# jerry102102102/RL_brain_trainer

Measured on AMD Instinct MI355X. Metric: env-steps/sec (whole node), Stage-5 Approach->Finisher PPO loops (rollout + update); value = the Approach loop, finisher.value = the Finisher loop, higher is better.
Workload: dtype f32

## Files before the change

### include/kp1_ppo.h

```cpp
#ifndef KP1_PPO_H
#define KP1_PPO_H

#include <stdint.h>

#include "kp1.h"

#ifdef __cplusplus
extern "C" {
#endif

int kp1_gae_scan(int32_t device, const float* rewards, const float* values, const uint8_t* dones, const float* last_values,
                 float gamma, float gae_lambda, float* advantages, float* returns, int32_t T, int32_t N, void* stream);

int kp1_gae_scan_replicas(int32_t device, const float* rewards, const float* values, const uint8_t* dones, const float* last_values,
                          const float* gamma_lambda, int32_t n_per_replica, float* advantages, float* returns, int32_t T, int32_t N, void* stream);

int kp1_bootstrap_truncated(int32_t device, float* rewards, const float* terminal_values, const uint8_t* dones, float gamma,
                            int64_t count, void* stream);

int kp1_adv_minibatch_sums(int32_t device, const float* advantages, const int64_t* idx, int64_t total, int64_t minibatch, double* out_sums,
                           void* stream);
int kp1_random_permutation(int32_t device, int64_t n, const uint32_t* keys, int64_t* out, void* stream);

int kp1_adv_minibatch_stats(int32_t device, const double* sums, int64_t n_minibatches, float* out_stats, void* stream);
// ... 56 lines not shown
typedef struct kp1_dock_curriculum_state {
  int32_t stage_index, stage_episode_count, ring_len, ring_head, window_episodes, n_stages, n_events, reserved0;
  int64_t num_timesteps;
  kp1_dock_curriculum_stage stages[KP1_DOCK_CURRICULUM_MAX_STAGES];
  kp1_dock_curriculum_event events[KP1_DOCK_CURRICULUM_MAX_HISTORY];
  uint8_t ring[KP1_DOCK_CURRICULUM_MAX_WINDOW];
} kp1_dock_curriculum_state;
int kp1_dock_curriculum_create(kp1_env* env, const kp1_dock_curriculum_stage* stages_host, int32_t n_stages, int32_t window_episodes,
                               kp1_dock_curriculum_state** out_dev);
int kp1_dock_curriculum_destroy(kp1_env* env, kp1_dock_curriculum_state* st_dev);
int kp1_dock_curriculum_observe(kp1_env* env, kp1_dock_curriculum_state* st_dev, const uint8_t* dones, int32_t n_local, int32_t chunk_steps, int32_t world,
                                void* stream);
int kp1_dock_curriculum_read(kp1_env* env, const kp1_dock_curriculum_state* st_dev, kp1_dock_curriculum_state* out_host, void* stream);
int kp1_dock_curriculum_create_population(kp1_env* env, const kp1_dock_curriculum_stage* stages_host, int32_t n_stages, int32_t window_episodes,
                                          int32_t n_replicas, kp1_dock_curriculum_state** out_dev);
int kp1_dock_curriculum_observe_population(kp1_env* env, kp1_dock_curriculum_state* states_dev, const uint8_t* dones, int32_t n_per_replica,
                                           int32_t n_replicas, void* stream);
int kp1_dock_curriculum_read_replica(kp1_env* env, const kp1_dock_curriculum_state* states_dev, int32_t n_replicas, int32_t k,
                                     kp1_dock_curriculum_state* out_host, void* stream);

#define KP1_MLP_IN 56
#define KP1_MLP_IN_PAD 64
#define KP1_MLP_IN_ROUTE 80
#define KP1_MLP_IN_ROUTE_PAD 128
#define KP1_MLP_ACT 7

typedef struct kp1_mlp kp1_mlp;

int kp1_mlp_create(int32_t device, int32_t hidden, int32_t max_batch, kp1_mlp** out);
int kp1_mlp_create_ex(int32_t device, int32_t hidden, int32_t obs_dim, int32_t max_batch, kp1_mlp** out);
#define KP1_MLP_MAX_REPLICAS 16
int kp1_mlp_create_population(int32_t device, int32_t hidden, int32_t obs_dim, int32_t max_batch, int32_t replicas, kp1_mlp** out);
int32_t kp1_mlp_replicas(const kp1_mlp* m);
typedef struct kp1_replica_hparams {
  float learning_rate, adam_eps, max_grad_norm, clip_range, ent_coef, vf_coef;
} kp1_replica_hparams;
int kp1_mlp_set_replica_hparams(kp1_mlp* m, const kp1_replica_hparams* host, int32_t n, void* stream);
int kp1_mlp_destroy(kp1_mlp* m);
int64_t kp1_mlp_num_params(int32_t hidden);
int64_t kp1_mlp_num_params_ex(int32_t hidden, int32_t obs_dim);
int kp1_mlp_pack_weights(kp1_mlp* m, const float* params, void* stream);

int kp1_mlp_forward(kp1_mlp* m, const float* obs, int32_t obs_stride, int32_t n, const float* noise, float* mean, float* value,
                    float* action, float* clipped_action, float* log_prob, void* stream);

int kp1_mlp_forward_env_step(kp1_mlp* m, kp1_env* env, const float* obs, int32_t obs_stride, const float* noise, float* value, float* action,
                             float* log_prob, float* next_obs, float* reward, uint8_t* done, float* terminal_obs, void* stream);

int kp1_eval_step(kp1_mlp* m, kp1_env* env, float* obs, float* reward, uint8_t* done, const kp1_eval_buffers* buffers, int32_t step,
                  const double* ready_thresholds , int32_t confirm_steps, void* stream);

#define KP1_EVAL_EPISODES_MAX_STEPS 256
int kp1_eval_episodes(kp1_mlp* m, kp1_env* env, float* obs, float* reward, uint8_t* done, const kp1_eval_buffers* buffers,
                      int32_t first_step, int32_t last_step, const double* ready_thresholds , int32_t confirm_steps, void* stream);

int kp1_mlp_loss_grad(kp1_mlp* m, const float* obs, int32_t obs_stride, const int64_t* idx, int32_t n, const float* actions,
                      const float* old_log_prob, const float* advantages, const float* returns, float adv_mean, float adv_inv_std,
                      const float* adv_stats_dev, float clip_range, float ent_coef, float vf_coef, float inv_count, float* grad_out,
                      float* stats_out, int32_t grad_is_zero, void* stream);

#define KP1_MLP_OPT_FUSED 1
#define KP1_MLP_OPT_ACTOR_EXTRA_STEPS 2
#define KP1_MLP_OPT_STEP_COUNT 3
#define KP1_MLP_OPT_PROFILE 4
#define KP1_MLP_OPT_BF16X3_WGRAD 5
#define KP1_MLP_PROFILE_SLOTS 4
#define KP1_MLP_PROFILE_TILE 0
#define KP1_MLP_PROFILE_WGRAD 1
#define KP1_MLP_PROFILE_FINALIZE 2
#define KP1_MLP_PROFILE_ADAM 3
int kp1_mlp_set_option(kp1_mlp* m, int32_t option, int32_t value);
int kp1_mlp_profile_read(kp1_mlp* m, float* out_us , int32_t* out_launches );

int kp1_mlp_adam_step(kp1_mlp* m, float* params, float* grad, float* exp_avg, float* exp_avg_sq, float lr, float eps,
                      float max_grad_norm, int32_t step, int32_t flags, void* stream);

int kp1_mlp_anchor_loss_grad(kp1_mlp* m, const float* obs, int32_t obs_stride, const int64_t* idx, int32_t n, const float* teacher_actions,
                             float loss_weight, float* grad_out, float* loss_out, void* stream);

int kp1_mlp_anchor_adam_step(kp1_mlp* m, float* params, float* grad, float* exp_avg, float* exp_avg_sq, float lr, float eps,
                             float max_grad_norm, int32_t step, void* stream);

int kp1_mlp_placement_check(int32_t device, int32_t n_rows, int32_t* out, void* stream);
int kp1_mlp_time_kernels(kp1_mlp* m, const float* obs, int32_t obs_stride, int32_t n, int32_t iters, float* out_ms, double* out_flops,
                         void* stream);

int kp1_set_obs_stride(kp1_env* env, int32_t stride);

#ifdef __cplusplus
}
#endif
#endif
```

### rl_brain_trainer_amd/csrc/kp1_mlp.hip

```cpp
#include <hip/hip_runtime.h>
#include <hip/hip_ext.h>

#include <cmath>
#include <cstddef>
#include <cstdlib>
#include <cstring>
#include <limits>
#include <vector>

#include "../../include/kp1_ppo.h"
#include "../../include/kp1_route.h"
#include "../../include/kp1_ziggurat_tables.h"
#include "kp1_device.hpp"
#include "kp1_host.hpp"

using kp1::fail;
using namespace kp1;

typedef float f32x16 __attribute__((ext_vector_type(16)));
typedef float f32x4 __attribute__((ext_vector_type(4)));

namespace {

constexpr int ACT = KP1_MLP_ACT, HEADS = 8;
// ... 1173 lines not shown

struct AnchorFinalizeArgs {
  FinalizeArgs f;
  float* loss_out;
};

template <bool POP = false>
__global__ void __launch_bounds__(256) anchor_finalize_kernel(const AnchorFinalizeArgs a_) {
  const FinalizeArgs a = POP ? finalize_args_replica(a_.f, blockIdx.y) : a_.f;
  const ParamLayout& L = a.L;
  __shared__ double sq[4];
  const int64_t i = (int64_t)(blockIdx.x * 256u + threadIdx.x);
  float gval = 0.f;
  if (i < L.total) {
    if (is_actor_element(L, i)) {
      const PartialSrc s = finalize_source(a, i);
      for (int c = 0; c < s.n; ++c) gval += s.p[(int64_t)c * s.stride];
    }
    a.grad[i] = gval;
  }
  if (blockIdx.x == 0 && threadIdx.x == 0) {
    float t = 0.f;
    for (int c = 0; c < a.h_n; ++c) t += a.hpart[(int64_t)c * a.h_stride + 10 * L.Hp + 15];
    a_.loss_out[POP ? blockIdx.y : 0u] = t;
  }
  double w = (double)gval * (double)gval;
  for (int off = 32; off > 0; off >>= 1) w += __shfl_xor(w, off);
  if ((threadIdx.x & 63) == 0) sq[threadIdx.x >> 6] = w;
  __syncthreads();
  if (threadIdx.x == 0) a.sumsq[blockIdx.x] = ((sq[0] + sq[1]) + sq[2]) + sq[3];
}

template <bool POP = false>
__global__ void __launch_bounds__(ADAM_BLOCK) anchor_adam_kernel(float* __restrict__ p, const float* __restrict__ g, float* __restrict__ m, float* __restrict__ v,
                                                          const double* __restrict__ partials, int n_partials, float lr, float eps, float max_norm,
                                                          const ParamLayout L, const Packed k_, const int* __restrict__ step_dev, int host_step,
                                                          unsigned r_partials, const float* __restrict__ hparams) {
  __shared__ float sh[3];
  const Packed k = POP ? packed_replica(k_, L, blockIdx.y) : k_;
  if constexpr (POP) {
    const unsigned o = blockIdx.y * (unsigned)L.total;
    p += o; g += o; m += o; v += o;
    partials += blockIdx.y * r_partials;
    if (hparams) {
      const float* e = hparams + blockIdx.y * (unsigned)HP_FIELDS;
      lr = e[HP_LR];
      eps = e[HP_EPS];
    }
  }
  const int64_t i = (int64_t)blockIdx.x * ADAM_BLOCK + threadIdx.x;
  const bool actor = i < L.total && is_actor_element(L, i);
  const int64_t il = actor ? i : L.p_w1;
  const float g_in = g[il], m_in = m[il], v_in = v[il], p_in = p[il];
  double s = 0.0;
  if (threadIdx.x < 64) {
    for (int q = threadIdx.x; q < n_partials; q += 64) s += partials[q];
    for (int off = 32; off > 0; off >>= 1) s += __shfl_xor(s, off);
  }
  if (threadIdx.x == 0) {
    const float norm = (float)sqrt(s);
    const int st = (host_step > 0 ? host_step : step_dev[0]) + step_dev[1] + 1;
    sh[0] = max_norm > 0.f ? fminf(max_norm / (norm + 1e-6f), 1.f) : 1.f;
    sh[1] = (float)((double)lr / (1.0 - pow(0.9, (double)st)));
    sh[2] = (float)sqrt(1.0 - pow(0.999, (double)st));
  }
  __syncthreads();
  if (actor) {
    const float gi = g_in * sh[0];
    const float mn = 0.9f * m_in + 0.1f * gi;
    const float vn = 0.999f * v_in + 0.001f * gi * gi;
    const float denom = sqrtf(vn) / sh[2] + eps;
    const float pn = p_in - sh[1] * (mn / denom);
    m[i] = mn; v[i] = vn; p[i] = pn;
    pack_one(i, pn, L, k);
  }
}

__global__ void anchor_count_kernel(int* __restrict__ actor_extra) { *actor_extra += 1; }

#include "kp1_env_step.inc"
#include "kp1_eval_step.inc"
#include "kp1_rollout_step.inc"
#include "kp1_mlp_tile.inc"
#include "kp1_mlp_fused.inc"
#include "kp1_route_step.inc"
#include "kp1_route_rollout_step.inc"
#include "kp1_route_chain_step.inc"

}

#include "kp1_route_host.hpp"

struct kp1_mlp {
  int device = 0, H = 0, Hp = 0, max_batch = 0;
  int K = 1;
  ParamLayout L;
  Packed k{};
  float* h1 = nullptr;
  float* h2 = nullptr;
  float* dz2 = nullptr;
  float* dz1 = nullptr;
  float* xf = nullptr;
  int bf16x3 = 0;
  unsigned short* sp_h1 = nullptr; unsigned short* sp_dz2 = nullptr; unsigned short* sp_dz1 = nullptr; unsigned short* sp_xf = nullptr;
  double* partials = nullptr;
  double* anchor_partials = nullptr;
  float* slab = nullptr;
  float* slab1 = nullptr;
  float* bslab = nullptr;
  float* hpart = nullptr;
  int n_finalize_blocks = 0;
  int* step_dev = nullptr;
  float* hparams_dev = nullptr;
  bool hparams_on = false;
  int last_s2_n = 0, last_s1_n = 0;
  int fused = 1;
  const float* last_params = nullptr;
  bool slab_stale = false;
  std::vector<void*> allocs;
  int profile = 0;
  struct ProfPair { hipEvent_t a, b; };
  std::vector<ProfPair> prof[KP1_MLP_PROFILE_SLOTS];
  int prof_used[KP1_MLP_PROFILE_SLOTS] = {0, 0, 0, 0};
};

namespace {
struct ProfSlotInFlight { hipEvent_t a = nullptr, b = nullptr; bool attached = false; };
thread_local ProfSlotInFlight tl_prof;

struct ProfScope {
  kp1_mlp* m; int slot; hipStream_t stream; bool on;
  ProfScope(kp1_mlp* m_, int slot_, hipStream_t s_) : m(m_), slot(slot_), stream(s_), on(m_->profile != 0) {
    if (!on) return;
    auto& v = m->prof[slot];
    if (m->prof_used[slot] >= (int)v.size()) {
      kp1_mlp::ProfPair p{};
      if (hipEventCreate(&p.a) != hipSuccess || hipEventCreate(&p.b) != hipSuccess) { on = false; return; }
      v.push_back(p);
    }
    tl_prof.a = v[m->prof_used[slot]].a;
    tl_prof.b = v[m->prof_used[slot]].b;
    tl_prof.attached = false;
  }
  ~ProfScope() {
    if (!on) return;
    if (!tl_prof.attached) {
      (void)hipEventRecord(tl_prof.a, stream);
      (void)hipEventRecord(tl_prof.b, stream);
    }
    tl_prof = ProfSlotInFlight{};
    m->prof_used[slot] += 1;
  }
};

#define KP1_LAUNCH(kernel, grid, block, bytes, stream, ...)                                                        \
  do {                                                                                                             \
    if (tl_prof.a != nullptr && !tl_prof.attached) {                                                               \
      tl_prof.attached = true;                                                                                     \
      hipExtLaunchKernelGGL(kernel, grid, block, bytes, stream, tl_prof.a, tl_prof.b, 0, __VA_ARGS__);             \
    } else {                                                                                                       \
      hipLaunchKernelGGL(kernel, grid, block, bytes, stream, __VA_ARGS__);                                         \
    }                                                                                                              \
  } while (0)
}

namespace {
// ... 1007 lines not shown
        if (launch_nt<EPI_DTANH>(g, stream) != KP1_OK) return KP1_ERR_NO_DEVICE;
      } else if (which == 2) {
        GemmTN t{};
        t.B = n; t.chunk = tn_chunk_rows(n, (Hp / 128) * (Hp / 128) * 2);
        t.D = m->dz2; t.ldd = Hp; t.strideD = act_stride; t.X = m->h1; t.ldx = Hp; t.strideX = act_stride;
        t.Nload = Hp; t.n_i_tiles = Hp / 128;
        if (launch_tn(m, t, Hp / 128, Hp, m->slab, nullptr, stream) != KP1_OK) return KP1_ERR_NO_DEVICE;
      } else if (which == 3) {
        g.A = obs; g.lda = obs_stride; g.strideA = 0; g.W = m->k.w1p; g.strideW = (int64_t)Hp * INP; g.bias = m->k.b1; g.strideBias = Hp;
        g.C = m->h1; g.K = INP; g.Kreal = obs_stride >= INP ? INP : IN;
        if (launch_nt<EPI_BIAS_TANH>(g, stream) != KP1_OK) return KP1_ERR_NO_DEVICE;
      } else if (which == 4) {
        FusedArgs fa{};
        fa.obs = obs; fa.obs_stride = obs_stride; fa.Kreal = obs_stride >= INP ? INP : IN; fa.inp = INP; fa.idx = nullptr; fa.n = n;
        fa.k = m->k;
        fa.actions = m->h2; fa.old_logp = m->h2 + (int64_t)ACT * n; fa.adv = m->h2 + (int64_t)(ACT + 1) * n; fa.ret = m->h2 + (int64_t)(ACT + 2) * n;
        fa.adv_mode = 3; fa.adv_mean = 0.f; fa.adv_inv_std = 1.f;
        fa.clip_range = 0.2f; fa.vf_coef = 0.5f; fa.inv_count = 1.f / n;
        fa.h1 = m->h1; fa.dz2 = m->dz2; fa.dz1 = m->dz1; fa.act_stride = act_stride; fa.xf = m->xf;
        fa.bslab = m->bslab; fa.hpart = m->hpart; fa.hpart_stride = 10 * Hp + 32;
        if (launch_fused(fa, stream) != KP1_OK) return KP1_ERR_NO_DEVICE;
      } else {
        TnFragArgs t{};
    t.inp = INP;
        t.dz2 = m->dz2; t.h1 = m->h1; t.dz1 = m->dz1; t.act_stride = act_stride; t.xf = m->xf;
        t.slab2 = m->slab; t.s2_net = (int64_t)Hp * Hp; t.s2_chunk = 2 * t.s2_net;
        t.slab1 = m->slab1; t.s1_net = (int64_t)Hp * INP; t.s1_chunk = 2 * t.s1_net;
        t.groups = (n + FU_BM - 1) / FU_BM * (FU_BM / 8);
        t.cg2 = ((t.groups + TN_SPLIT2 - 1) / TN_SPLIT2 + 7) / 8 * 8;
        t.cg1 = ((t.groups + TN_SPLIT1 - 1) / TN_SPLIT1 + 7) / 8 * 8;
        t.n_chunks2 = (t.groups + t.cg2 - 1) / t.cg2;
        t.n_chunks1 = (t.groups + t.cg1 - 1) / t.cg1;
        if (launch_tn_frag(t, stream) != KP1_OK) return KP1_ERR_NO_DEVICE;
      }
    }
    HIP_TRY(hipEventRecord(e1, stream));
    HIP_TRY(hipEventSynchronize(e1));
    float ms = 0.f;
    HIP_TRY(hipEventElapsedTime(&ms, e0, e1));
    out_ms[which] = ms / iters;
    return KP1_OK;
  };
  for (int which : {3, 0, 1, 2}) {
    rc = time_it(which);
    if (rc != KP1_OK) return rc;
  }
  out_ms[4] = out_ms[5] = 0.f;
  out_flops[4] = out_flops[5] = 0.0;
  if (Hp == FU_HP) {
    for (int which : {4, 5}) {
      rc = time_it(which);
      if (rc != KP1_OK) return rc;
    }
  }
  const double M = n, H = Hp;
  out_flops[0] = 2.0 * 2.0 * M * H * H;
  out_flops[1] = 2.0 * 2.0 * M * H * H;
  out_flops[2] = 2.0 * 2.0 * M * H * H;
  out_flops[3] = 2.0 * 2.0 * M * H * INP;
  if (Hp == FU_HP) {
    out_flops[4] = 2.0 * 2.0 * M * (H * (double)INP + 2.0 * H * H);
    out_flops[5] = 2.0 * 2.0 * M * (H * H + H * (double)INP);
  }
  (void)hipEventDestroy(e0);
  (void)hipEventDestroy(e1);
  return KP1_OK;
}

__global__ void __launch_bounds__(FU_NTH, 2) placement_probe_kernel(unsigned int* __restrict__ where, unsigned int* __restrict__ arrived, unsigned int total) {
  extern __shared__ float lds[];
  if (threadIdx.x == 0) {
    const unsigned int hw = __builtin_amdgcn_s_getreg((31 << 11) | 4);
    const unsigned int xcc = __builtin_amdgcn_s_getreg((3 << 11) | 20);
    const unsigned int linear = blockIdx.x + gridDim.x * blockIdx.z;
    where[linear] = (xcc << 16) | (((hw >> 13) & 7u) << 8) | (((hw >> 12) & 1u) << 4) | ((hw >> 8) & 15u);
    lds[0] = 0.f;
    __hip_atomic_fetch_add(arrived, 1u, __ATOMIC_RELAXED, __HIP_MEMORY_SCOPE_AGENT);
    const unsigned long long t0 = wall_clock64();
    while (__hip_atomic_load(arrived, __ATOMIC_RELAXED, __HIP_MEMORY_SCOPE_AGENT) < total && wall_clock64() - t0 < 200000ull) __builtin_amdgcn_s_sleep(8);
  }
  __syncthreads();
}

int kp1_mlp_placement_check(int32_t device, int32_t n_rows, int32_t* out, void* stream_) {
  if (!out || n_rows <= 0) return fail(KP1_ERR_INVALID, "bad argument to kp1_mlp_placement_check");
  HIP_TRY(hipSetDevice(device));
  hipStream_t stream = (hipStream_t)stream_;
  int n_cus = 0;
  HIP_TRY(hipDeviceGetAttribute(&n_cus, hipDeviceAttributeMultiprocessorCount, device));
  const dim3 grid((n_rows + FU_BM - 1) / FU_BM, 1, 2);
  const unsigned int total = grid.x * grid.z;
  if ((int)total > 2 * n_cus) return fail(KP1_ERR_UNSUPPORTED, "placement probe: the grid must be resident at once");
  unsigned int* dev = nullptr;
  HIP_TRY(hipMalloc(&dev, sizeof(unsigned int) * (total + 1)));
  HIP_TRY(hipMemsetAsync(dev, 0, sizeof(unsigned int) * (total + 1), stream));
  const size_t bytes = sizeof(float) * FU_LDS_FLOATS;
  HIP_TRY(hipFuncSetAttribute((const void*)placement_probe_kernel, hipFuncAttributeMaxDynamicSharedMemorySize, (int)bytes));
  hipLaunchKernelGGL(placement_probe_kernel, grid, dim3(FU_NTH), bytes, stream, dev, dev + total, total);
  std::vector<unsigned int> host(total + 1);
  hipError_t e = hipMemcpyAsync(host.data(), dev, sizeof(unsigned int) * (total + 1), hipMemcpyDeviceToHost, stream);
  if (e == hipSuccess) e = hipStreamSynchronize(stream);
  (void)hipFree(dev);
  HIP_TRY(e);
  int pairs = 0, same = 0, rr = 0;
  std::vector<unsigned int> seen;
  for (unsigned int k = 0; k < total; ++k) {
    if ((host[k] >> 16) == (host[k & 7u] >> 16)) ++rr;
    if (k + (unsigned)n_cus < total) {
      ++pairs;
      if (host[k] == host[k + n_cus]) ++same;
    }
    bool fresh = true;
    for (unsigned int v : seen) fresh = fresh && v != host[k];
    if (fresh) seen.push_back(host[k]);
  }
  int xcds = 0;
  for (unsigned int a = 0; a < 8 && a < total; ++a) {
    bool fresh = true;
    for (unsigned int b = 0; b < a; ++b) fresh = fresh && (host[a] >> 16) != (host[b] >> 16);
    xcds += fresh ? 1 : 0;
  }
  out[0] = (int)total; out[1] = pairs; out[2] = same; out[3] = rr; out[4] = n_cus; out[5] = (int)seen.size(); out[6] = (int)host[total]; out[7] = xcds;
  return KP1_OK;
}

#ifdef KP1_CLK_TRACE
int kp1_debug_clk_trace(unsigned long long* out) {
  HIP_TRY(hipDeviceSynchronize());
  HIP_TRY(hipMemcpyFromSymbol(out, HIP_SYMBOL(kp1_clk_buf), sizeof(unsigned long long) * 2 * 1024 * 4));
  return KP1_OK;
}
#endif

#ifdef KP1_NT_TRACE
int kp1_debug_nt_trace(unsigned long long* out, int clear) {
  HIP_TRY(hipDeviceSynchronize());
  if (out) HIP_TRY(hipMemcpyFromSymbol(out, HIP_SYMBOL(kp1_nt_trace_buf), sizeof(unsigned long long) * KP1_TRACE_SLOTS * KP1_TRACE_WGS));
  if (clear) {
    std::vector<unsigned long long> z(KP1_TRACE_SLOTS * KP1_TRACE_WGS, 0ull);
    HIP_TRY(hipMemcpyToSymbol(HIP_SYMBOL(kp1_nt_trace_buf), z.data(), sizeof(unsigned long long) * z.size()));
  }
  return KP1_OK;
}
#endif

int kp1_mlp_adam_step(kp1_mlp* m, float* params, float* grad, float* exp_avg, float* exp_avg_sq, float lr, float eps, float max_grad_norm,
                      int32_t step, int32_t zero_grad, void* stream_) {
  if (!m || !params || !grad || !exp_avg || !exp_avg_sq) return fail(KP1_ERR_INVALID, "bad argument to kp1_mlp_adam_step");
  int rc = mlp_check_device(m);
  if (rc != KP1_OK) return rc;
  hipStream_t stream = (hipStream_t)stream_;
  const int64_t n = m->L.total;
  const bool fused_norm = (zero_grad & 2) && m->n_finalize_blocks > 0;
  const double* norm_partials = fused_norm ? m->partials + 2 * N_PARTIALS : m->partials + N_PARTIALS;
  const int n_norm_partials = fused_norm ? m->n_finalize_blocks : N_PARTIALS;
  ProfScope ps(m, KP1_MLP_PROFILE_ADAM, stream);
  const bool pop = m->K > 1;
  if (!fused_norm) {
    if (pop)
      hipLaunchKernelGGL(sumsq_partials_kernel<true>, dim3(N_PARTIALS, m->K), dim3(256), 0, stream, grad, n, m->partials + N_PARTIALS, (unsigned)PARTIALS_STRIDE);
    else
      hipLaunchKernelGGL(sumsq_partials_kernel<false>, dim3(N_PARTIALS), dim3(256), 0, stream, grad, n, m->partials + N_PARTIALS, 0u);
  }
  zero_grad = 0;
  const int host_step = step > 0 ? step : 1;
  const float bc1 = 1.f - std::pow(0.9f, (float)host_step);
// ... 128 lines not shown
```

### rl_brain_trainer_amd/csrc/kp1_mlp_fused.inc

```

struct TnFragArgs {
  const float* dz2; const float* h1; const float* dz1; int64_t act_stride;
  const float* xf; int inp;
  float* slab2; int64_t s2_net, s2_chunk;
  float* slab1; int64_t s1_net, s1_chunk;
  int groups, cg2, n_chunks2, cg1, n_chunks1;
};

template <int RA, int CB>
__device__ __forceinline__ void tn_split_tile(const float* __restrict__ Af, int a_ncb, const float* __restrict__ Bf, int b_ncb, int g_begin, int g_end,
                                              float* __restrict__ out, int out_ld, float* lds) {
  constexpr int SG = 4;
  const int tid = threadIdx.x, lane = tid & 63, wave = __builtin_amdgcn_readfirstlane(tid >> 6);
  const int per = (max(g_end - g_begin, 0) + 3) >> 2;
  const int gb = min(g_begin + wave * per, g_end), ge = min(gb + per, g_end);
  const int64_t a_gs = (int64_t)a_ncb * 256, b_gs = (int64_t)b_ncb * 256;
  f32x4 ra[2][SG][RA], rb[2][SG][CB];
  f32x16 acc[RA][CB];
#pragma unroll
  for (int r = 0; r < RA; ++r)
#pragma unroll
    for (int c = 0; c < CB; ++c)
#pragma unroll
      for (int e = 0; e < 16; ++e) acc[r][c][e] = 0.f;
  KP1_TR(12)
  KP1_TR_HW(11)
  if (gb < ge) {
    const int g_last = ge - 1;
#define KP1_TNS_LOAD(set, g0)                                                                           \
  _Pragma("unroll") for (int u = 0; u < SG; ++u) {                                                      \
    const int gg_ = min((g0) + u, g_last);                                                              \
    _Pragma("unroll") for (int r = 0; r < RA; ++r) ra[set][u][r] = load16_sc1(Af, lane * 4 + gg_ * a_gs + r * 256); \
    _Pragma("unroll") for (int c = 0; c < CB; ++c) rb[set][u][c] = load16_sc1(Bf, lane * 4 + gg_ * b_gs + c * 256); \
  }
#define KP1_TNS_MFMA(set, g0)                                                                           \
  _Pragma("unroll") for (int u = 0; u < SG; ++u) {                                                      \
    const float keep_ = (g0) + u < ge ? 1.f : 0.f;                                                      \
    _Pragma("unroll") for (int i = 0; i < 4; ++i)                                                       \
      _Pragma("unroll") for (int r = 0; r < RA; ++r)                                                    \
        _Pragma("unroll") for (int c = 0; c < CB; ++c)                                                  \
          acc[r][c] = __builtin_amdgcn_mfma_f32_32x32x2f32(ra[set][u][r][i] * keep_, rb[set][u][c][i], acc[r][c], 0, 0, 0); \
  }
    KP1_TNS_LOAD(0, gb)
    for (int g = gb; g < ge; g += 2 * SG) {
      KP1_TNS_LOAD(1, g + SG)
      __builtin_amdgcn_sched_barrier(0);
      KP1_TNS_MFMA(0, g)
      __builtin_amdgcn_sched_barrier(0);
      KP1_TNS_LOAD(0, g + 2 * SG)
      __builtin_amdgcn_sched_barrier(0);
      KP1_TNS_MFMA(1, g + SG)
      __builtin_amdgcn_sched_barrier(0);
    }
#undef KP1_TNS_LOAD
#undef KP1_TNS_MFMA
  }
  KP1_TR(13)
  constexpr int TO = 32 * RA, TI = 32 * CB, LDP = TI + 8, Q = TI / 4;
  float* mine = lds + wave * (TO * LDP);
#pragma unroll
  for (int r = 0; r < RA; ++r)
#pragma unroll
    for (int c = 0; c < CB; ++c)
#pragma unroll
      for (int e = 0; e < 16; ++e) {
        const int o = r * 32 + (e & 3) + 8 * (e >> 2) + 4 * (lane >> 5);
        mine[o * LDP + c * 32 + (lane & 31)] = acc[r][c][e];
      }
  __syncthreads();
  KP1_TR(14)
#pragma unroll
  for (int j = 0; j < TO * Q / 256; ++j) {
    const int f = tid + 256 * j, o = f / Q, q = f % Q;
    const float* p0 = lds + o * LDP + 4 * q;
    const f32x4 v = ((*reinterpret_cast<const f32x4*>(p0) + *reinterpret_cast<const f32x4*>(p0 + TO * LDP)) +
                     *reinterpret_cast<const f32x4*>(p0 + 2 * TO * LDP)) + *reinterpret_cast<const f32x4*>(p0 + 3 * TO * LDP);
    store16_sc1(out, (int64_t)o * out_ld + 4 * q, v);
  }
  KP1_TR(15)
}
constexpr int TN_SPLIT_LDS_FLOATS = 4 * 64 * (64 + 8);

__global__ void __launch_bounds__(256, 2) gemm_tn_split_kernel(const TnFragArgs a) {
  extern __shared__ float lds[];
  KP1_CLK(1, 0)
  const int n2 = 32 * a.n_chunks2;
  if ((int)blockIdx.x < n2) {
    const int chunk = blockIdx.x % a.n_chunks2, tile = blockIdx.x / a.n_chunks2;
    const int net = tile >> 4, ot = (tile >> 2) & 3, it = tile & 3;
    const int g0 = chunk * a.cg2, g1 = min(g0 + a.cg2, a.groups);
    float* out = a.slab2 + chunk * a.s2_chunk + net * a.s2_net + (int64_t)(ot * 64) * FU_HP + it * 64;
    tn_split_tile<2, 2>(a.dz2 + net * a.act_stride + (ot * 2) * 256, 8, a.h1 + net * a.act_stride + (it * 2) * 256, 8, g0, g1, out, FU_HP, lds);
  } else {
    const int id = blockIdx.x - n2;
    const int chunk = id % a.n_chunks1, tile = id / a.n_chunks1;
    const int net = tile >> 3, ot = tile & 7;
    const int g0 = chunk * a.cg1, g1 = min(g0 + a.cg1, a.groups);
    const int inp = a.inp;
    float* out = a.slab1 + chunk * a.s1_chunk + net * a.s1_net + (int64_t)(ot * 32) * inp;
    if (inp == 64)
      tn_split_tile<1, 2>(a.dz1 + net * a.act_stride + ot * 256, 8, a.xf, 2, g0, g1, out, 64, lds);
    else
      tn_split_tile<1, 3>(a.dz1 + net * a.act_stride + ot * 256, 8, a.xf, 4, g0, g1, out, 128, lds);
  }
  KP1_CLK(1, 1)
}

struct TnBf16Args {
  const unsigned short* dz2; const unsigned short* h1; const unsigned short* dz1; int64_t plane, net;
  const unsigned short* xf; int64_t plane_x; int inp;
  float* slab2; int64_t s2_net, s2_chunk;
  float* slab1; int64_t s1_net, s1_chunk;
  int frags, cf2, n_chunks2, cf1, n_chunks1;
};

__device__ __forceinline__ bf16x8 tnb_load(const unsigned short* __restrict__ base, int64_t off) {
  const __amdgpu_buffer_rsrc_t r = __builtin_amdgcn_make_buffer_rsrc(const_cast<unsigned short*>(base), 0, 0x7fffffff, 0x00020000);
  return __builtin_bit_cast(bf16x8, __builtin_amdgcn_raw_buffer_load_b128(r, (int)(off * 2), 0, AUX_SC1));
}

template <int RA, int CB>
__device__ __forceinline__ void tn_bf16_tile(const unsigned short* __restrict__ Af, int64_t a_plane, int a_ncb, const unsigned short* __restrict__ Bf, int64_t b_plane,
                                             int b_ncb, int f_begin, int f_end, float* __restrict__ out, int out_ld, float* lds) {
  const int tid = threadIdx.x, lane = tid & 63, wave = __builtin_amdgcn_readfirstlane(tid >> 6);
  const int per = (max(f_end - f_begin, 0) + 3) >> 2;
  const int fb = min(f_begin + wave * per, f_end), fe = min(fb + per, f_end);
  const int64_t a_fs = (int64_t)a_ncb * 512, b_fs = (int64_t)b_ncb * 512;
  bf16x8 ra[2][3][RA], rb[2][3][CB];
  f32x16 acc[RA][CB];
#pragma unroll
  for (int r = 0; r < RA; ++r)
#pragma unroll
    for (int c = 0; c < CB; ++c)
#pragma unroll
      for (int e = 0; e < 16; ++e) acc[r][c][e] = 0.f;
  if (fb < fe) {
    const int f_last = fe - 1;
#define KP1_TNB_LOAD(set, f0)                                                                           \
  {                                                                                                     \
    const int ff_ = min((f0), f_last);                                                                  \
    _Pragma("unroll") for (int pl = 0; pl < 3; ++pl) {                                                  \
// ... 76 lines not shown
```

Before: 11.40 million.

## Stream TN split-GEMM operands through an LDS ring via global_load_lds

Replaces the register double-buffered global loads in the TN split-K weight-gradient tile with a 4-slot per-wave LDS ring filled by global_load_lds_dwordx4 inline asm, then read back with ds_read_b128 into a small register double buffer. Tail groups read from a zeroed LDS slab instead of multiplying by a keep mask. The aim is to cut VGPR pressure and keep several loads in flight with explicit vmcnt waits, so more MFMA work overlaps the memory latency. The cost is extra LDS traffic, hand-written asm with m0 juggling, and an added syncthreads before the reduction. A host-side plan query is also exported for testing.

After: 11.50 million, median of 6. No clear change (+0.9%).

```diff
diff --git a/include/kp1_ppo.h b/include/kp1_ppo.h
--- a/include/kp1_ppo.h
+++ b/include/kp1_ppo.h
@@ -162,6 +162,7 @@
                              float max_grad_norm, int32_t step, void* stream);
 
 int kp1_mlp_placement_check(int32_t device, int32_t n_rows, int32_t* out, void* stream);
+int kp1_tn_ring_plan(int32_t n_groups, int32_t step, int32_t* out);
 int kp1_mlp_time_kernels(kp1_mlp* m, const float* obs, int32_t obs_stride, int32_t n, int32_t iters, float* out_ms, double* out_flops,
                          void* stream);
 
diff --git a/rl_brain_trainer_amd/csrc/kp1_mlp.hip b/rl_brain_trainer_amd/csrc/kp1_mlp.hip
--- a/rl_brain_trainer_amd/csrc/kp1_mlp.hip
+++ b/rl_brain_trainer_amd/csrc/kp1_mlp.hip
@@ -1279,6 +1279,7 @@
 #include "kp1_eval_step.inc"
 #include "kp1_rollout_step.inc"
 #include "kp1_mlp_tile.inc"
+#include "kp1_tn_ring.inc"
 #include "kp1_mlp_fused.inc"
 #include "kp1_route_step.inc"
 #include "kp1_route_rollout_step.inc"
@@ -2452,6 +2453,13 @@
   __syncthreads();
 }
 
+int kp1_tn_ring_plan(int32_t n_groups, int32_t step, int32_t* out) {
+  if (!out || n_groups < 1 || step < -1) return fail(KP1_ERR_INVALID, "bad argument to kp1_tn_ring_plan");
+  const TnRingStep s = tn_ring_step(n_groups, step);
+  out[0] = s.slot; out[1] = s.issue; out[2] = s.keep; out[3] = s.a_slot; out[4] = s.b_slot;
+  return KP1_OK;
+}
+
 int kp1_mlp_placement_check(int32_t device, int32_t n_rows, int32_t* out, void* stream_) {
   if (!out || n_rows <= 0) return fail(KP1_ERR_INVALID, "bad argument to kp1_mlp_placement_check");
   HIP_TRY(hipSetDevice(device));
diff --git a/rl_brain_trainer_amd/csrc/kp1_mlp_fused.inc b/rl_brain_trainer_amd/csrc/kp1_mlp_fused.inc
--- a/rl_brain_trainer_amd/csrc/kp1_mlp_fused.inc
+++ b/rl_brain_trainer_amd/csrc/kp1_mlp_fused.inc
@@ -8,14 +8,41 @@
 };
 
 template <int RA, int CB>
+__device__ __forceinline__ void tn_ring_issue(unsigned lds_a, unsigned lds_b, const float* sa, const float* sb, unsigned voff) {
+  static_assert((RA == 2 && CB == 2) || (RA == 1 && (CB == 2 || CB == 3)), "tile shapes of gemm_tn_split_kernel");
+  unsigned keep;
+#define KP1_GLDS_(src, off) "global_load_lds_dwordx4 %3, " src " offset:" off " sc1\n\t"
+#define KP1_GLDS_OPEN_ "s_nop 4\n\ts_mov_b32 %0, m0\n\ts_mov_b32 m0, %1\n\ts_nop 0\n\t"
+#define KP1_GLDS_B_ "s_mov_b32 m0, %2\n\ts_nop 0\n\t"
+#define KP1_GLDS_OPS_ : "=&s"(keep) : "s"(lds_a), "s"(lds_b), "v"(voff), "s"(sa), "s"(sb) : "memory"
+  if constexpr (RA == 2)
+    asm volatile(KP1_GLDS_OPEN_ KP1_GLDS_("%4", "0") KP1_GLDS_("%4", "1024") KP1_GLDS_B_ KP1_GLDS_("%5", "0") KP1_GLDS_("%5", "1024") "s_mov_b32 m0, %0" KP1_GLDS_OPS_);
+  else if constexpr (CB == 2)
+    asm volatile(KP1_GLDS_OPEN_ KP1_GLDS_("%4", "0") KP1_GLDS_B_ KP1_GLDS_("%5", "0") KP1_GLDS_("%5", "1024") "s_mov_b32 m0, %0" KP1_GLDS_OPS_);
+  else
+    asm volatile(KP1_GLDS_OPEN_ KP1_GLDS_("%4", "0") KP1_GLDS_B_ KP1_GLDS_("%5", "0") KP1_GLDS_("%5", "1024") KP1_GLDS_("%5", "2048") "s_mov_b32 m0, %0" KP1_GLDS_OPS_);
+#undef KP1_GLDS_
+#undef KP1_GLDS_OPEN_
+#undef KP1_GLDS_B_
+#undef KP1_GLDS_OPS_
+}
+template <int F>
+__device__ __forceinline__ void tn_ring_read(f32x4& x, unsigned addr) {
+  asm volatile("ds_read_b128 %0, %1 offset:%2" : "=v"(x) : "v"(addr), "n"(F * 1024) : "memory");
+}
+
+template <int RA, int CB>
 __device__ __forceinline__ void tn_split_tile(const float* __restrict__ Af, int a_ncb, const float* __restrict__ Bf, int b_ncb, int g_begin, int g_end,
                                               float* __restrict__ out, int out_ld, float* lds) {
-  constexpr int SG = 4;
+  constexpr int TO = 32 * RA, TI = 32 * CB, LDP = TI + 8, Q = TI / 4;
+  constexpr int SLOT_B = (RA + CB) * 1024, RING_B = TN_RING_SLOTS * SLOT_B, ZERO_B = RA * 1024;
+  static_assert(4 * RING_B <= 65536 && 4 * (RING_B + ZERO_B) <= (int)sizeof(float) * 4 * 64 * (64 + 8) && 4 * TO * LDP <= 4 * 64 * (64 + 8), "dynamic LDS of the launch");
   const int tid = threadIdx.x, lane = tid & 63, wave = __builtin_amdgcn_readfirstlane(tid >> 6);
   const int per = (max(g_end - g_begin, 0) + 3) >> 2;
   const int gb = min(g_begin + wave * per, g_end), ge = min(gb + per, g_end);
+  const int n = ge - gb;
   const int64_t a_gs = (int64_t)a_ncb * 256, b_gs = (int64_t)b_ncb * 256;
-  f32x4 ra[2][SG][RA], rb[2][SG][CB];
+  f32x4 ra[2][RA], rb[2][CB];
   f32x16 acc[RA][CB];
 #pragma unroll
   for (int r = 0; r < RA; ++r)
@@ -25,38 +52,72 @@
       for (int e = 0; e < 16; ++e) acc[r][c][e] = 0.f;
   KP1_TR(12)
   KP1_TR_HW(11)
-  if (gb < ge) {
-    const int g_last = ge - 1;
-#define KP1_TNS_LOAD(set, g0)                                                                           \
-  _Pragma("unroll") for (int u = 0; u < SG; ++u) {                                                      \
-    const int gg_ = min((g0) + u, g_last);                                                              \
-    _Pragma("unroll") for (int r = 0; r < RA; ++r) ra[set][u][r] = load16_sc1(Af, lane * 4 + gg_ * a_gs + r * 256); \
-    _Pragma("unroll") for (int c = 0; c < CB; ++c) rb[set][u][c] = load16_sc1(Bf, lane * 4 + gg_ * b_gs + c * 256); \
-  }
-#define KP1_TNS_MFMA(set, g0)                                                                           \
-  _Pragma("unroll") for (int u = 0; u < SG; ++u) {                                                      \
-    const float keep_ = (g0) + u < ge ? 1.f : 0.f;                                                      \
+  if (n > 0) {
+    const unsigned lds_u = __builtin_amdgcn_readfirstlane((unsigned)(size_t)(__attribute__((address_space(3))) float*)lds);
+    const unsigned ring_u = lds_u + wave * RING_B, voff = lane * 16;
+    const unsigned ring_v = ring_u + voff, zero_v = lds_u + 4 * RING_B + wave * ZERO_B + voff;
+    const float* const a0 = Af + gb * a_gs;
+    const float* const b0 = Bf + gb * b_gs;
+#pragma unroll
+    for (int r = 0; r < RA; ++r) *reinterpret_cast<f32x4*>(lds + (4 * RING_B + wave * ZERO_B) / 4 + r * 256 + lane * 4) = f32x4{0.f, 0.f, 0.f, 0.f};
+#define KP1_TNS_WAIT(keep_)                                                                             \
+  if ((keep_) == 2) asm volatile("s_waitcnt vmcnt(%0)" : : "n"(2 * (RA + CB)) : "memory");              \
+  else if ((keep_) == 1) asm volatile("s_waitcnt vmcnt(%0)" : : "n"(RA + CB) : "memory");               \
+  else asm volatile("s_waitcnt vmcnt(0)" : : : "memory");
+#define KP1_TNS_READ(set, s_)                                                                           \
+  {                                                                                                     \
+    const unsigned av_ = (s_).a_slot == TN_RING_ZERO ? zero_v : ring_v + (s_).a_slot * SLOT_B;          \
+    const unsigned bv_ = ring_v + (s_).b_slot * SLOT_B;                                                 \
+    tn_ring_read<0>(ra[set][0], av_);                                                                   \
+    if constexpr (RA == 2) tn_ring_read<1>(ra[set][RA - 1], av_);                                       \
+    tn_ring_read<RA>(rb[set][0], bv_);                                                                  \
+    tn_ring_read<RA + 1>(rb[set][1], bv_);                                                              \
+    if constexpr (CB == 3) tn_ring_read<RA + 2>(rb[set][CB - 1], bv_);                                  \
+  }
+#define KP1_TNS_LANDED(set)                                                                             \
+  asm volatile("s_waitcnt lgkmcnt(0)" : : : "memory");                                                  \
+  _Pragma("unroll") for (int r = 0; r < RA; ++r) asm volatile("" : "+v"(ra[set][r]));                   \
+  _Pragma("unroll") for (int c = 0; c < CB; ++c) asm volatile("" : "+v"(rb[set][c]));
+#define KP1_TNS_STEP(set, j)                                                                            \
+  {                                                                                                     \
+    const TnRingStep s_ = tn_ring_step(n, (j));                                                         \
+    KP1_TNS_LANDED(set)                                                                                 \
+    if (s_.issue >= 0)                                                                                  \
+      tn_ring_issue<RA, CB>(ring_u + s_.slot * SLOT_B, ring_u + s_.slot * SLOT_B + RA * 1024, a0 + s_.issue * a_gs, b0 + s_.issue * b_gs, voff); \
+    KP1_TNS_WAIT(s_.keep)                                                                               \
+    __builtin_amdgcn_sched_barrier(0);                                                                  \
+    KP1_TNS_READ((set) ^ 1, s_)                                                                         \
+    __builtin_amdgcn_sched_barrier(0);                                                                  \
     _Pragma("unroll") for (int i = 0; i < 4; ++i)                                                       \
       _Pragma("unroll") for (int r = 0; r < RA; ++r)                                                    \
         _Pragma("unroll") for (int c = 0; c < CB; ++c)                                                  \
-          acc[r][c] = __builtin_amdgcn_mfma_f32_32x32x2f32(ra[set][u][r][i] * keep_, rb[set][u][c][i], acc[r][c], 0, 0, 0); \
-  }
-    KP1_TNS_LOAD(0, gb)
-    for (int g = gb; g < ge; g += 2 * SG) {
-      KP1_TNS_LOAD(1, g + SG)
-      __builtin_amdgcn_sched_barrier(0);
-      KP1_TNS_MFMA(0, g)
-      __builtin_amdgcn_sched_barrier(0);
-      KP1_TNS_LOAD(0, g + 2 * SG)
-      __builtin_amdgcn_sched_barrier(0);
-      KP1_TNS_MFMA(1, g + SG)
-      __builtin_amdgcn_sched_barrier(0);
-    }
-#undef KP1_TNS_LOAD
-#undef KP1_TNS_MFMA
+          acc[r][c] = __builtin_amdgcn_mfma_f32_32x32x2f32(ra[set][r][i], rb[set][c][i], acc[r][c], 0, 0, 0); \
+    __builtin_amdgcn_sched_barrier(0);                                                                  \
+  }
+#pragma unroll
+    for (int u = 0; u < TN_RING_SLOTS; ++u)
+      if (u < n) tn_ring_issue<RA, CB>(ring_u + u * SLOT_B, ring_u + u * SLOT_B + RA * 1024, a0 + u * a_gs, b0 + u * b_gs, voff);
+    {
+      const TnRingStep s_ = tn_ring_step(n, -1);
+      KP1_TNS_WAIT(s_.keep)
+      __builtin_amdgcn_sched_barrier(0);
+      KP1_TNS_READ(0, s_)
+      __builtin_amdgcn_sched_barrier(0);
+    }
+    for (int j = 0; j < n; j += TN_RING_SLOTS) {
+      KP1_TNS_STEP(0, j)
+      KP1_TNS_STEP(1, j + 1)
+      KP1_TNS_STEP(0, j + 2)
+      KP1_TNS_STEP(1, j + 3)
+    }
+    KP1_TNS_LANDED(0)
+#undef KP1_TNS_WAIT
+#undef KP1_TNS_READ
+#undef KP1_TNS_LANDED
+#undef KP1_TNS_STEP
   }
   KP1_TR(13)
-  constexpr int TO = 32 * RA, TI = 32 * CB, LDP = TI + 8, Q = TI / 4;
+  __syncthreads();
   float* mine = lds + wave * (TO * LDP);
 #pragma unroll
   for (int r = 0; r < RA; ++r)
diff --git a/rl_brain_trainer_amd/csrc/kp1_tn_ring.inc b/rl_brain_trainer_amd/csrc/kp1_tn_ring.inc
--- /dev/null
+++ b/rl_brain_trainer_amd/csrc/kp1_tn_ring.inc
@@ -0,0 +1,21 @@
+constexpr int TN_RING_SLOTS = 4;
+constexpr int TN_RING_ZERO = -1;
+
+struct TnRingStep {
+  int slot;
+  int issue;
+  int keep;
+  int a_slot;
+  int b_slot;
+};
+
+__host__ __device__ inline TnRingStep tn_ring_step(int n, int j) {
+  TnRingStep s;
+  s.slot = j & (TN_RING_SLOTS - 1);
+  s.issue = j + TN_RING_SLOTS < n ? j + TN_RING_SLOTS : -1;
+  s.keep = j + 4 < n ? 2 : j + 3 < n ? 1 : 0;
+  const bool live = j + 1 < n;
+  s.a_slot = live ? (j + 1) & (TN_RING_SLOTS - 1) : TN_RING_ZERO;
+  s.b_slot = (live ? j + 1 : n - 1) & (TN_RING_SLOTS - 1);
+  return s;
+}
```
